# noce2/FluidFramework

Measured on AMD Instinct MI355X. Metric: sequenced merge-tree ops applied/sec (node) at 100k docs; bit-exact text+props, higher is better.
Workload: dtype int32; 1 GPU; c3: 100000 docs/GPU x 10000 sequenced ops, 8 writers, refSeq lag <= 64, insert 0.5 / remove 0.3 / annotate 0.2; docs_total=100000, docs_per_gpu=100000, ops_per_doc=10000, parallelism=doc-shard x1

## Files before the change

### fluidframework_amd/__init__.py

```python
import ctypes

import numpy as np

from . import _native
from .wire import CHECKSUM_DTYPE, OP_DTYPE, Batch, Interner

__all__ = ["MergeTreeBatch", "DeviceBatch", "Batch", "Interner", "DeltaLogOverflow"]


class DeltaLogOverflow(RuntimeError):

    def __init__(self, msg, records):
        super().__init__(msg)
        self.records = records


class PinnedArray:

    def __init__(self, lib, n, dtype):
        dt = np.dtype(dtype)
        nbytes = max(int(n), 1) * dt.itemsize
        self.lib = lib
        self.p = lib.mt_host_alloc(nbytes)
        if not self.p:
# ... 331 lines not shown

    def upload(self, a):
        return DeviceBatch(self, a)

    def generate(self, cfg, doc_base=0, trace=None, ops_per_doc=None, doc_ids=None):
        c = _native.gen_cfg(cfg)
        if ops_per_doc is not None or doc_ids is not None:
            lens = None if ops_per_doc is None else np.ascontiguousarray(ops_per_doc, dtype=np.int32)
            ids = None if doc_ids is None else np.ascontiguousarray(doc_ids, dtype=np.int32)
            for x in (lens, ids):
                if x is not None and x.shape != (self.n_docs,):
                    raise ValueError("ops_per_doc / doc_ids: one per document")
            b = self.lib.mt_generate_docs(self.h, ctypes.byref(c), doc_base, _native.ptr(lens), _native.ptr(ids),
                                          _native.ptr(trace))
        else:
            b = self.lib.mt_generate(self.h, ctypes.byref(c), doc_base, _native.ptr(trace))
        if not b:
            raise RuntimeError(f"mt_generate failed: {self.lib.mt_last_error(self.h).decode()}")
        return DeviceBatch(self, None, handle=b)

    def generated_seeds(self, cfg, doc_base=0, doc_ids=None):
        c = _native.gen_cfg(cfg)
        ids = None if doc_ids is None else np.ascontiguousarray(doc_ids, dtype=np.int32)
        off = np.zeros(self.n_docs + 1, dtype=np.int64)
        self._check(self.lib.mt_generated_seeds_docs(self.h, ctypes.byref(c), doc_base, _native.ptr(ids),
                                                     _native.ptr(off), None), "mt_generated_seeds")
        seed = np.zeros(max(int(off[-1]), 1), dtype=np.uint16)
        self._check(self.lib.mt_generated_seeds_docs(self.h, ctypes.byref(c), doc_base, _native.ptr(ids),
                                                     _native.ptr(off), _native.ptr(seed)), "mt_generated_seeds")
        return off, seed

    def sync(self):
        self._check(self.lib.mt_sync(self.h), "mt_sync")

    def last_hbm_docs(self):
        out = np.zeros(8, dtype=np.uint32)
        self._check(self.lib.mt_last_hbm_docs(self.h, _native.ptr(out)), "mt_last_hbm_docs")
        return dict(total=int(out[0]), spilled=int(out[1]), segments=int(out[2]), blocks=int(out[3]), heap=int(out[4]),
                    text=int(out[5]), props=int(out[6]), at_load=int(out[7]))

    def last_paged_peaks(self):
        out = np.zeros(5, dtype=np.uint32)
        self._check(self.lib.mt_last_paged_peaks(self.h, _native.ptr(out)), "mt_last_paged_peaks")
        return dict(pages=int(out[0]), unsettled=int(out[1]), heap=int(out[2]), segments=int(out[3]),
                    tight_handovers=int(out[4]))

    def last_zamboni(self):
        out = np.zeros(2, dtype=np.uint32)
        self._check(self.lib.mt_last_zamboni(self.h, _native.ptr(out)), "mt_last_zamboni")
        packs = np.zeros(1, dtype=np.uint32)
        self._check(self.lib.mt_last_zamboni_packs(self.h, _native.ptr(packs)), "mt_last_zamboni_packs")
        return {"in_place": int(out[0]), "fallback": int(out[1]), "in_place_packs": int(packs[0])}

    def last_grown(self):
        out = np.zeros(6, dtype=np.uint32)
        self._check(self.lib.mt_last_grown(self.h, _native.ptr(out)), "mt_last_grown")
        return dict(zip(["grown", "rounds", "in_big_region", "pages", "unsettled", "heap"], (int(x) for x in out)))

    def last_kernel_ms(self):
        return float(self.lib.mt_last_kernel_ms(self.h))

    def set_stream_priority(self, priority):
        self._check(self.lib.mt_set_stream_priority(self.h, int(priority)), "mt_set_stream_priority")

    def last_load_ms(self):
        return float(self.lib.mt_last_load_ms(self.h))

    def status(self):
        out = np.zeros(self.n_docs, dtype=np.int32)
        self._check(self.lib.mt_get_status(self.h, _native.ptr(out)), "mt_get_status")
        return out

    def get_length(self, doc):
        out = ctypes.c_uint32()
        self._check(self.lib.mt_get_length(self.h, doc, ctypes.byref(out)), "mt_get_length")
        return out.value

    def get_text(self, doc):
        n = ctypes.c_uint32()
        self._check(self.lib.mt_get_text(self.h, doc, None, 0, ctypes.byref(n)), "mt_get_text")
        buf = np.zeros(max(n.value, 1), dtype=np.uint16)
        self._check(self.lib.mt_get_text(self.h, doc, _native.ptr(buf), n.value, ctypes.byref(n)),
                    "mt_get_text")
        return buf[: n.value].tobytes().decode("utf-16-le", errors="surrogatepass")

    def _text_queries(self, docs, start, end, placeholder):
        if isinstance(placeholder, str):
            units = np.frombuffer(placeholder.encode("utf-16-le", errors="surrogatepass"), dtype=np.uint16)
            if len(units) > 1:
                raise ValueError("get_texts: the placeholder is empty or one UTF-16 unit")
            placeholder = int(units[0]) if len(units) else 0
        if docs is not None:
            docs = np.ascontiguousarray(docs, dtype=np.uint32).reshape(-1)
        n = len(docs) if docs is not None else self.n_docs
        if start is not None:
            start = np.ascontiguousarray(np.broadcast_to(np.asarray(start, dtype=np.int32), (n,)))
        if end is not None:
            end = np.asarray([-1 if e is None else e for e in end] if isinstance(end, (list, tuple)) else end)
            end = np.ascontiguousarray(np.broadcast_to(end.astype(np.int32), (n,)))
        return n, docs, start, end, int(placeholder)

    def get_texts_raw(self, docs=None, start=None, end=None, placeholder=""):
        n, docs, start, end, mu = self._text_queries(docs, start, end, placeholder)
        off = np.zeros(n + 1, dtype=np.int64)
        args = (self.h, n, _native.ptr(docs), _native.ptr(start), _native.ptr(end), mu, _native.ptr(off))
        self._check(self.lib.mt_get_texts(*args, None, 0), "mt_get_texts")
# ... 390 lines not shown
```

### fluidframework_amd/_native.py

```python
import ctypes
import os

import numpy as np

from .wire import CHECKSUM_DTYPE, OP_DTYPE

HERE = os.path.dirname(os.path.abspath(__file__))
MT_E_INVALID, MT_E_HIP, MT_E_NOMEM, MT_E_NODEVICE, MT_E_OVERFLOW, MT_E_STALE_VIEW = -1, -2, -3, -4, -5, -6
LIB_PATH = os.environ.get("MT_LIB_PATH") or os.path.join(HERE, "libmtreplay.so")


class MtOptions(ctypes.Structure):
    _fields_ = [("device", ctypes.c_int32), ("seg_capacity", ctypes.c_int32),
                ("block_capacity", ctypes.c_int32), ("heap_capacity", ctypes.c_int32),
                ("text_capacity", ctypes.c_int32), ("props_capacity", ctypes.c_int32),
                ("delta_log_capacity", ctypes.c_int32), ("lds_seg_capacity", ctypes.c_int32),
                ("page_capacity", ctypes.c_int32), ("page_heap_capacity", ctypes.c_int32),
                ("unsettled_capacity", ctypes.c_int32), ("uid_capacity", ctypes.c_int32),
                ("lds_page_capacity", ctypes.c_int32), ("lds_unsettled_capacity", ctypes.c_int32),
                ("lds_page_heap_capacity", ctypes.c_int32), ("lds_narrow_overlap", ctypes.c_int32),
                ("delta_log_mode", ctypes.c_int32), ("live_client", ctypes.c_int32),
                ("live_group_capacity", ctypes.c_int32), ("paged_slices", ctypes.c_int32),
                ("segment_ordinals", ctypes.c_int32), ("overlap_arena_capacity", ctypes.c_int32)]

# ... 7 lines not shown


REGEN_DTYPE = np.dtype([("kind", "<i4"), ("pos1", "<i4"), ("pos2", "<i4"), ("local_seq", "<i4"),
                        ("text_off", "<u4"), ("text_len", "<u4"), ("props_off", "<u4"), ("flags", "<u4")])


SEG_HIT_DTYPE = np.dtype([("row", "<i4"), ("uid", "<u4"), ("position", "<i4"), ("offset", "<i4"),
                          ("local_position", "<i4"), ("length", "<i4"), ("seq", "<i4"), ("client", "<i4"),
                          ("removed_seq", "<i4"), ("removed_client", "<i4"), ("marker_ref_type", "<i4"),
                          ("flags", "<u4")])
MT_HIT_HOST = 1


class MtGenCfg(ctypes.Structure):
    _fields_ = [("seed", ctypes.c_uint32), ("ops", ctypes.c_int32), ("writers", ctypes.c_int32),
                ("lag", ctypes.c_int32), ("seed_len", ctypes.c_int32), ("text_max", ctypes.c_int32),
                ("n_keys", ctypes.c_int32), ("n_values", ctypes.c_int32),
                ("max_keys_per_op", ctypes.c_int32), ("_pad", ctypes.c_int32),
                ("p_insert", ctypes.c_uint64), ("p_insert_remove", ctypes.c_uint64),
                ("p_newline", ctypes.c_uint64), ("p_len_continue", ctypes.c_uint64),
                ("p_insert_props", ctypes.c_uint64), ("p_null", ctypes.c_uint64)]


_P, _I, _U32, _U64 = ctypes.c_void_p, ctypes.c_int, ctypes.c_uint32, ctypes.c_uint64
SIGNATURES = [
    ("mt_create", _P, [_U32, _P]),
    ("mt_destroy", None, [_P]),
    ("mt_last_error", ctypes.c_char_p, [_P]),
    ("mt_num_docs", _U32, [_P]),
    ("mt_load_initial_text", _I, [_P, _P, _P]),
    ("mt_start_collaboration", _I, [_P, _P, _P]),
    ("mt_reset", _I, [_P]),
    ("mt_apply_ops", _I, [_P, _P, _P, _U64, _P, _U64, _P, _U64]),
    ("mt_load_snapshots", _I, [_P, _P, _P, _P, _U64, _P, _U64, _P, _U64, _P, _P]),
    ("mt_extract_snapshots", _I, [_P, _P, _P, _P, _P, _P, _P]),
    ("mt_snapshots_upload", _P, [_P, _P, _P, _P, _U64, _P, _U64, _P, _U64, _P, _P]),
    ("mt_snapshots_upload_range", _P, [_P, _U32, _U32, _P, _P, _P, _U64, _P, _U64, _P, _U64, _P, _P]),
    ("mt_snapshots_load_async", _I, [_P, _P]),
    ("mt_snapshots_free", None, [_P]),
    ("mt_batch_upload", _P, [_P, _P, _P, _U64, _P, _U64, _P, _U64]),
    ("mt_batch_apply_async", _I, [_P, _P]),
    ("mt_batch_num_ops", _U64, [_P]),
    ("mt_batch_free", None, [_P]),
    ("mt_host_alloc", ctypes.c_void_p, [ctypes.c_uint64]),
    ("mt_host_free", None, [ctypes.c_void_p]),
    ("mt_sync", _I, [_P]),
    ("mt_last_kernel_ms", ctypes.c_float, [_P]),
    ("mt_set_stream_priority", ctypes.c_int, [_P, ctypes.c_int]),
    ("mt_last_load_ms", ctypes.c_float, [_P]),
    ("mt_last_hbm_docs", _I, [_P, _P]),
    ("mt_last_paged_peaks", _I, [_P, _P]),
    ("mt_last_zamboni", _I, [_P, _P]),
    ("mt_last_zamboni_packs", _I, [_P, _P]),
    ("mt_last_grown", _I, [_P, _P]),
    ("mt_generate", _P, [_P, _P, _U32, _P]),
    ("mt_generate_docs", _P, [_P, _P, _U32, _P, _P, _P]),
    ("mt_generated_seeds_docs", _I, [_P, _P, _U32, _P, _P, _P]),
    ("mt_generated_seeds", _I, [_P, _P, _U32, _P, _P]),
    ("mt_batch_sizes", _I, [_P, _P, _P, _P]),
    ("mt_batch_download", _I, [_P, _P, _P, _P, _P]),
    ("mt_get_status", _I, [_P, _P]),
    ("mt_get_length", _I, [_P, _U32, _P]),
    ("mt_get_text", _I, [_P, _U32, _P, _U32, _P]),
    ("mt_get_texts", _I, [_P, _U32, _P, _P, _P, ctypes.c_uint16, _P, _P, _U64]),
    ("mt_get_texts_device", _I, [_P, _U32, _P, _P, _P, ctypes.c_uint16, _P, _P, _U64]),
    ("mt_last_text_ms", _I, [_P, _P]),
    ("mt_get_prop_runs", _I, [_P, _U32, _P, _U32, _P, _P, _U32, _P]),
    ("mt_get_prop_runs_bulk", _I, [_P, _U32, _P, _P, _P, _P, _P, _P, _U64, _P, _U64]),
    ("mt_get_prop_runs_bulk_device", _I, [_P, _U32, _P, _P, _P, _P, _P, _P, _U64, _P, _U64]),
    ("mt_last_props_ms", _I, [_P, _P]),
    ("mt_get_segments", _I, [_P, _U32, _P, _U32, _P, _P, _U32, _P]),
    ("mt_get_segment_props", _I, [_P, _U32, _U32, _P, _U32, _P]),
    ("mt_get_all_segment_props", _I, [_P, _U32, _P, ctypes.c_uint64, _P]),
    ("mt_get_overlap_arena", _I, [_P, _U32, _P]),
    ("mt_get_delta_log", _I, [_P, _U32, _P, _U32, _P]),
    ("mt_delta_log_reset", _I, [_P]),
    ("mt_debug_raw", _I, [_P, _U32, _P, _U32, _P, _P]),
    ("mt_debug_prof", _I, [_P, _P, _I]),
    ("mt_maintenance_counts", _I, [_P, _P]),
    ("mt_checksums", _I, [_P, _P]),
    ("mt_checksums_device", _I, [_P, _P]),
    ("mt_regenerate_pending", _I, [_P, _U32, _P, _U32, _P, _P, _U32, _P, _U32]),
    ("mt_pending_counts", _I, [_P, _P]),
    ("mt_debug_heap", _I, [_P, _U32, _P, _U32, _P, _P, _U32, _P]),
    ("mt_get_containing_segment", _I, [_P, _U32, ctypes.c_int32, ctypes.c_int32, ctypes.c_int32, _P, _P, _U32]),
    ("mt_get_segment_by_uid", _I, [_P, _U32, _U32, ctypes.c_int32, ctypes.c_int32, _P, _P, _U32]),
    ("mt_get_view_lengths", _I, [_P, _U32, _P, _P, _P, _P]),
    ("mt_locate_segments", _I, [_P, _U32, _P, _P, _P, _P, _P]),
    ("mt_locate_uids", _I, [_P, _U32, _P, _P, _P, _P, _P]),
    ("mt_locate_segments_device", _I, [_P, _U32, _P, _P, _P, _P, _P]),
    ("mt_locate_uids_device", _I, [_P, _U32, _P, _P, _P, _P, _P]),
    ("mt_get_view_lengths_bulk", _I, [_P, _U32, _P, _P, _P, _P]),
    ("mt_resolve_remote_positions", _I, [_P, _U32, _P, _P, _P, _P, _P]),
    ("mt_last_locate", _I, [_P, _P, _P]),
]

_lib = None


def load():
    global _lib
    if _lib is not None:
        return _lib
    if not os.path.exists(LIB_PATH):
        raise RuntimeError(f"HIP replay library missing: {LIB_PATH} (run __graft_entry__.build())")
    lib = ctypes.CDLL(LIB_PATH)
# ... 21 lines not shown
```

### fluidframework_amd/csrc/mt_device.h

```cpp
#pragma once
#include <hip/hip_runtime.h>
#include <stdint.h>

#include "../../include/mt_types.h"

#define MT_WAVE 64
#define MT_LV 8
#define MT_MAXN 8
#define MT_HALF 4
#define MT_GRAN 256
#define MT_STATS_WORDS 20
#define MT_ZAMBONI 2
#define MT_KMAX 8
#define MT_PREC (1 + 2 * MT_KMAX)
#define MT_RSEQ_NONE ((int32_t)0x80000000)
#define MT_MARKER_BIT 0x80000000u
#define MT_SCOUR_UNDEF ((int8_t)-1)
#define MT_DOC_RETRY 100

typedef unsigned long long u64;
typedef int v4i __attribute__((ext_vector_type(4)));
typedef unsigned v4u __attribute__((ext_vector_type(4)));
typedef int v2i __attribute__((ext_vector_type(2)));

struct DocHdr {
    int32_t n_seg, depth, heap_n, cur_seq;
    int32_t min_seq, text_top, text_half, props_top;
    int32_t props_half, next_uid, status, dlog_n;
    int32_t n_blk[MT_LV];
    u64 delta_hash;
    int32_t n_ops, pad0;
    int32_t pad[8];
};
static_assert(sizeof(DocHdr) == 128, "DocHdr size");

struct PageMeta {
    uint8_t nseg, nblk;
    uint16_t flg2;
    uint32_t bc;
    int32_t obs;
};
static_assert(sizeof(PageMeta) == 12, "PageMeta size");
static __host__ __device__ inline int pm_bcnt(const PageMeta &m, int q) { return (int)((m.bc >> (4 * q)) & 15u); }
static __host__ __device__ inline int8_t pm_flg(const PageMeta &m, int q) { return (int8_t)((int)((m.flg2 >> (2 * q)) & 3u) - 1); }
#define MT_OSLOTS 64
#define MT_OSLOT_USE 63
#define MT_OVF_BIT (1ull << 63)
#define MT_OVF_HDR 12
static __host__ __device__ inline int mt_ovf_mid(int OA) { return MT_OVF_HDR + (((OA - MT_OVF_HDR) / 2) & ~7); }
#define MT_OVF_ARENA 8192
#define MT_OSLOT_FREE 0x7FFFFFFF
#define MT_PG_SLOTS 64
#define MT_PG_OLB 32
#define HDR_PAGED 0
#define HDR_NPAGES 1
#define HDR_UTN 2
#define HDR_DIAG 3
#define HDR_MSPLIT 4
#define HDR_MAPPEND 5
#define HDR_MUNLINK 6
#define HDR_DLOG_OVF 7

struct PagedRegion {
    v4i *A;
// ... 243 lines not shown
```

### fluidframework_amd/csrc/mt_kernels.h

```cpp
#pragma once
#include "../../include/mt_replay.h"
#include "mt_paged.h"

__device__ static void init_doc_hdr(const DevState &st, int doc, int len) {
    DocHdr h;
    memset(&h, 0, sizeof(h));
    h.depth = 1;
    h.n_blk[0] = 1;
    h.text_top = len;
    h.props_top = 1;
    h.next_uid = 2;
    h.delta_hash = MT_FNV_OFF;
    h.status = len > st.T ? MT_DOC_CAPACITY : 0;
    const size_t S = st.S;
    if (len > 0) {
        h.n_seg = 1;
        st.segA[doc * S] = v4i{len, 0, MT_RSEQ_NONE, pack_cli(-1, 0)};
        st.segO[doc * S] = 0ull;
        st.segB[doc * S] = v4u{0u, 0u, 1u, 0u};
        if (st.segP) {
            u64 *w = (u64 *)(st.segP + doc * S);
            w[0] = w[1] = w[2] = w[3] = 0ull;
        }
    }
// ... 363 lines not shown
    for (int t = 1; t <= g.n && d.status == 0; t++) {
        int r, c, msn;
        gen_pick(g, cfg, t, r, c, msn);
        d.ocs = oslot_of(d, c);
        int vsum = 0;
        for (int base = 0; base < d.n; base += MT_WAVE) {
            const int i = base + lane();
            v4i a;
            u64 o;
            load_ao(d, i, i < d.n, a, o);
            vsum += i < d.n ? view_len(a, o, r, c, d.ocs) : 0;
        }
        const int len = wave_sum(vsum);
        if (dbg_len && lane() == 0) {
            int32_t *q = dbg_len + (g.ob + (t - 1)) * 4;
            q[0] = len;
            q[1] = d.n;
            q[2] = r;
            q[3] = c;
        }
        OpIn in;
        gen_op(g, cfg, t, r, c, msn, len, in, ops_out, text_out, props_out, doc);
        apply_op(d, in, gt, gp);
    }
    gen_end(g, used_out, doc);
    if (T::kLds && d.status == MT_DOC_RETRY) {
        if (lane() == 0) st.retry[doc] = 1;
        return;
    }
    if (lane() == 0) {
        if (d.status) fail_out[doc] = d.status;
        if (!T::kLds) st.retry[doc] = 0;
    }
    store_doc(d, st, doc);
}

template <class T>
__device__ __forceinline__ void pg_peaks(const DevState &st, PagedDoc<T> &pd, int pk_ut, int pk_heap) {
    const int np = nbr(pd.up, 1);
    int ns = 0;
    for (int q = lane(); q < np; q += MT_WAVE) ns += pm_nseg(pd, pd.up.dir[q]);
    ns = wave_sum(ns);
    if (lane() == 0) {
        atomicMax(st.stats + 8, (uint32_t)np);
        atomicMax(st.stats + 9, (uint32_t)pk_ut);
        atomicMax(st.stats + 10, (uint32_t)pk_heap);
        atomicMax(st.stats + 11, (uint32_t)ns);
        if constexpr (pg_zinplace<T>()) {
            const uint32_t zi = pg_zcount(pd)[0], zf = pg_zcount(pd)[1], zp = pg_zcount(pd)[2];
            if (zi) atomicAdd(st.stats + 16, zi);
            if (zf) atomicAdd(st.stats + 17, zf);
            if (zp) atomicAdd(st.stats + 18, zp);
        }
    }
}
#ifndef MT_PAGED_WAVES
#define MT_PAGED_WAVES 3
#endif
#ifndef MT_HM_WAVES
#define MT_HM_WAVES 2
#endif
#ifndef MT_FULL_WAVES
#define MT_FULL_WAVES 2
#endif
#ifndef MT_PACKED_WAVES
#define MT_PACKED_WAVES 2
#endif
template <class T> constexpr int paged_waves() {
    return T::kHM ? MT_HM_WAVES
                  : (T::kMayGrow ? MT_FULL_WAVES : (T::kPacked ? MT_PACKED_WAVES : MT_PAGED_WAVES));
}
#if MT_PAGED_WAVES > 0
#define MT_PAGED_WPE __attribute__((amdgpu_waves_per_eu(paged_waves<T>())))
#else
#define MT_PAGED_WPE
#endif
template <class T>
__device__ __forceinline__ void pg_handover(const DevState &st, int doc, int64_t k, const PagedCaps &pc) {
    if (lane() == 0) {
        st.retry[doc] = pc.tight ? 2 : 3;
        st.resume[doc] = k;
        atomicAdd(st.stats + (pc.tight ? 12 : 13), 1u);
    }
}
struct PagedSlice {
    int64_t ops;
    int skip_lo, skip_hi, cnt_lo, cnt_hi;
};

template <class T>
__global__ void __launch_bounds__(MT_WAVE) MT_PAGED_WPE k_replay_paged(DevState st, const mt_op_rec *ops,
                                                          const int64_t *off, const uint16_t *tin,
                                                          const uint32_t *pin, int use_resume, PagedCaps pc_arg,
                                                          PagedSlice sl) {
    extern __shared__ __attribute__((aligned(16))) uint8_t smem_raw[];
    LDS_AS uint8_t *smem = (LDS_AS uint8_t *)smem_raw;
    const PagedCaps pc = eff_caps<T>(pc_arg);
    const int di = blockIdx.x;
    if (di >= st.n_docs) return;
    if (di >= sl.skip_lo && di < sl.skip_hi) return;
    const int doc = doc_at(st, di);
    if (st.retry[doc] != pc.stage) return;
    if (lane() == 0 && di >= sl.cnt_lo && di < sl.cnt_hi) atomicAdd(st.stats, 1u);
    const PagedLayout L = paged_layout(pc.PP, pc.PH, pc.UT, 0, (int)sizeof(typename T::O_v), T::kPacked, T::kHM);
    const int64_t k0 = use_resume ? st.resume[doc] : off[doc];
    const int64_t kend = off[doc + 1];
// ... 220 lines not shown
```

### fluidframework_amd/csrc/mt_paged.h

```cpp
#pragma once
#include "mt_engine.h"

#ifdef MT_PROF
#define PG_T0(k) const unsigned long long _pt##k = __builtin_amdgcn_s_memtime();
#define PG_T1(k)                                                         \
    if (lane() == 0) {                                                   \
        pd.w.prof[k] += __builtin_amdgcn_s_memtime() - _pt##k;           \
        pd.w.prof[64 + k] += 1ull;                                       \
    }
#define PG_CNT(k)                                                        \
    if (lane() == 0) pd.w.prof[64 + k] += 1ull;
#else
#define PG_T0(k)
#define PG_T1(k)
#define PG_CNT(k)
#endif

template <class T> struct PagedDoc {
    DocT<T> w;
    DocT<T> up;
    LDS_AS PageMeta *meta;
    GLB_AS PageMeta *gmeta;
    LDS_AS int *pvl;
    LDS_AS int *cob;
// ... 13 lines not shown
    GLB_AS uint16_t *goS;
    GLB_AS uint16_t *goL;
    int doc;
    int PP, PH, UT, UM;
    int PPh;
    int ut_n;
    int cur;
    int cur_pos;
    int dirty;
    int tdirty;
    int uid_lo;
    int vvalid, vr, vc;
    int zuid, zpv;
    GLB_AS uint16_t *govf;
    int ovf_top, ovf_last, OA;
    int ovf_maxn, ovf_half;
    uint32_t ovf_made;
    int ovf_peak;
    int press;
    int wgrow, opbound;
    LDS_AS int *sob;
    int sob_ch;
    int wnb, wobs;
};

struct PagedCaps {
    int PP, PH, UT;
    int tight;
    int stage;
    int narrow;
    int grow;
    int packed;
};

#define PW_B 16
#define MT_PK_MASKS 256

struct PagedLayout {
    uint32_t offWA, offWB, offWO, offWcnt, offWflg, offWends, offWscr, offWnb;
    uint32_t offUcnt, offUnb, offDir, offMeta, offCob, offHeap, offUpage, offUA, offUO, offGen, offProf,
        total;
};
static __host__ __device__ inline PagedLayout paged_layout(int PP, int PH, int UT, int gen_words, int ob,
                                                           bool packed = false, bool hm = false) {
    PagedLayout L;
    uint32_t o = 0;
    L.offWA = o; o += 16u * MT_PG_SLOTS;
    L.offWB = o; o += 16u * MT_PG_SLOTS;
    L.offWO = o; o += (uint32_t)ob * MT_PG_SLOTS;
    L.offUA = o; o += (packed ? 12u : 16u) * UT;
    o = (o + 7u) & ~7u;
    L.offUO = o; o += packed ? 8u * MT_PK_MASKS + MT_PK_MASKS / 8 : ((((uint32_t)ob * UT) + 7u) & ~7u);
    L.offHeap = o; o += 8u * (PH + 1);
    L.offMeta = o; o += hm ? 0u : (uint32_t)sizeof(PageMeta) * PP + 12u;
    L.offUpage = o; o += packed ? 0u : (2u * UT + 3u) & ~3u;
    L.offCob = o; o += hm ? 8u * (uint32_t)((PP + 63) / 64) + 4u * 64 : 4u * PP;
    L.offWscr = o; o += 64u * 4;
    L.offWnb = o; o += MT_LV * 4;
    L.offUnb = o; o += MT_LV * 4;
    L.offGen = o; o += 4u * gen_words;
    L.offDir = o; o += 2u * PP;
    L.offWends = o; o += 2u * PW_B;
    L.offWcnt = o; o += (uint32_t)MT_LV * PW_B;
    L.offWflg = o; o += PW_B;
    L.offUcnt = o; o += (uint32_t)(pcnt_bytes(PP) - PP);
#ifdef MT_PROF
    o = (o + 7u) & ~7u;
    L.offProf = o; o += 128u * 8;
#else
    L.offProf = 0;
#endif
    L.total = (o + 15u) & ~15u;
    return L;
}

TD PagedDoc<T> &pdoc(DocT<T> &w) { return *reinterpret_cast<PagedDoc<T> *>(&w); }
template <class T> __device__ __forceinline__ PagedCaps eff_caps(PagedCaps pc) {
    if constexpr (T::kPP > 0) pc.PP = T::kPP;
    if constexpr (T::kPH > 0) pc.PH = T::kPH;
    if constexpr (T::kUT > 0) pc.UT = T::kUT;
    return pc;
}
TD void pg_fail_cap(DocT<T> &w, int cause) {
    if (w.status == 0) w.cap_cause = cause;
    fail(w, MT_DOC_CAPACITY);
}
__device__ __forceinline__ PageMeta pm_load(const LDS_AS PageMeta *m) {
    PageMeta r;
    r.nseg = m->nseg;
    r.nblk = m->nblk;
    r.flg2 = m->flg2;
    r.bc = m->bc;
    r.obs = m->obs;
    return r;
}
__device__ __forceinline__ int pm_bcnt_l(const LDS_AS PageMeta *m, int q) { return (int)((m->bc >> (4 * q)) & 15u); }
__device__ __forceinline__ int8_t pm_flg_l(const LDS_AS PageMeta *m, int q) {
    return (int8_t)((int)((m->flg2 >> (2 * q)) & 3u) - 1);
}
TD int pm_nseg(const PagedDoc<T> &pd, int pg) {
    if constexpr (T::kHM) {
        gsync_rd();
        return pd.gmeta[pg].nseg;
    } else {
        return pd.meta[pg].nseg;
    }
}
TD int pm_nblk(const PagedDoc<T> &pd, int pg) {
    if constexpr (T::kHM) {
// ... 1177 lines not shown
            pd.gO[(size_t)npg * MT_PG_SLOTS + t] = o;
            pd.gB[(size_t)npg * MT_PG_SLOTS + t] = b;
            const uint32_t uid = b.z & ~MT_MARKER_BIT;
            if (uid < (uint32_t)pd.UM) pd.gumap[uid] = (uint16_t)npg;
            ol = obs_len(a);
            add = unsettled<T>(a, w.min_seq);
        }
        const u64 am = ballot(add);
        if (pd.ut_n + __popcll(am) > pd.UT) {
            pg_fail_cap(w, 8);
            return;
        }
        const int mi = tab_midx(pd, add && o != 0);
        if (mi < 0) {
            pg_fail_cap(w, 8);
            return;
        }
        if (add) tab_put(pd, pd.ut_n + __popcll(am & ((1ull << lane()) - 1ull)), c0 + m, a, o, mi);
        pd.ut_n += __popcll(am);
        const int obs = wave_sum(ol);
        const bool vb = lane() >= blo && lane() < bhi;
        pm_set_blocks(pd, npg, lane() - blo, vb, bcnt, bflg);
        if (lane() == 0) {
            pm_set_ns(pd, npg, s_hi - s_lo, bhi - blo);
            pm_set_obs(pd, npg, obs);
        }
        wsync<T>();
    }
    for (int j = 0; j < nch; j++) {
        const int pg = uni(up.dir[c0 + j]);
        if (lane() == 0) pm_set_ns(pd, pg, 0, 0);
        wsync<T>();
    }
    blk_replace(up, 1, c0, nch, k, base, extra);
    if (up.status) {
        pg_fail_cap(w, 7);
        return;
    }
    for (int m = 0; m < k; m++)
        if (lane() == 0) up.dir[c0 + m] = (uint16_t)newp[m];
    if (lane() == 0) lvl(up, 2)[P] = (uint8_t)k;
    wsync<T>();
    pg_cob_rebuild(pd);
    int top_l = 2, top_b = P;
    if (k < MT_HALF && 3 < up.depth) pack_counts(up, 2, P, top_l, top_b);
    if (up.status) {
        if (w.status == 0) w.cap_cause = up.cap_cause;
        fail(w, MT_DOC_INTERNAL);
        return;
    }
    if (ordon(w)) ord_canon(up, top_l, top_b);
}

TD LDS_AS uint32_t *pg_zcount(PagedDoc<T> &pd) { return (LDS_AS uint32_t *)(pd.meta + pd.PP); }
template <class T> constexpr bool pg_zinplace() {
#ifdef MT_NO_ZINPLACE
    return false;
#else
    return !T::kLog && !T::kHM && !T::kLive;
#endif
}
template <class T> constexpr bool pg_zpack() {
#ifdef MT_NO_ZPACK
    return false;
#else
    return pg_zinplace<T>();
#endif
}
__device__ __forceinline__ int lane_push(int v, int dst) { return __builtin_amdgcn_ds_permute(dst << 2, v); }
TD bool pg_pack_inplace(PagedDoc<T> &pd, int pg, v4i a, v4u b, const ScourPlan &pl, uint32_t bc, int q, int bstart) {
    DocT<T> &w = pd.w;
    const int k = lane();
    const int n = uni(pm_nseg(pd, pg)), nb = uni(pm_nblk(pd, pg));
    const int cnt = pm_bc_of(bc, q);
    const int keep = __popcll(pl.m_surv);
    const int n1 = n - (cnt - keep);
    if (nb > 8) return true;
    const bool in = k >= bstart && k < bstart + cnt;
    const u64 below = (1ull << k) - 1ull;
    const ScourGroups g1 = scour_groups(a, in, pl.m_join, pl.m_surv);
    v4i a1 = a;
    v4u b1 = b;
    if (g1.m_grp) {
        const uint32_t lastw = (uint32_t)__shfl((int)b.w, g1.gend & (MT_WAVE - 1), MT_WAVE);
        if ((g1.m_grp >> k) & 1ull) {
            a1.x = g1.glen;
            b1.w = lastw & (SEGF_NL_KNOWN | SEGF_NL);
        }
    }
    const int d1 = k < bstart ? k
                   : !in      ? k - (cnt - keep)
                   : ((pl.m_surv >> k) & 1ull) ? bstart + __popcll(pl.m_surv & below) : MT_WAVE - 1;
    a1 = v4i{lane_push(a1.x, d1), lane_push(a1.y, d1), lane_push(a1.z, d1), lane_push(a1.w, d1)};
    b1 = v4u{(uint32_t)lane_push((int)b1.x, d1), (uint32_t)lane_push((int)b1.y, d1),
             (uint32_t)lane_push((int)b1.z, d1), (uint32_t)lane_push((int)b1.w, d1)};
    const int src1 = lane_push(k, d1);
    const bool in2 = k < n1;
    int start2 = 0;
    {
        int st = 0;
        for (int j = 0; j < nb; j++) {
            if (k >= st) start2 = st;
            st += j == q ? keep : pm_bc_of(bc, j);
        }
    }
    bool nl2;
    const ScourPlan p2 = scour_plan(w, a1, b1, in2, false, start2, nl2);
// ... 272 lines not shown
    int start;
    int ostart;
    int pos = pg_find(pd, op.pos1, false, start, ostart);
    if constexpr (T::kLog) {
        const int np = nbr(pd.up, 1);
        if (pos < 0 && slen == 0 && np > 0 && !(op.flags & MT_F_LOAD)) {
            pos = np - 1;
            const int lp = uni((int)pd.up.dir[pos]);
            start -= pg_page_view(pd, pos);
            ostart -= uni(pm_obs(pd, lp));
        }
    }
    if (pos < 0) {
        if (slen == 0) {
            if (op.flags & MT_F_LOAD) return;
            Cb cb = cb_begin(w, op.seq, MT_OP_INSERT);
            cb.n = 1;
            cb_log(w, -1);
            cb_log(w, 0);
            cb.h = fnv_u64(cb.h, fnv_u32(fnv_u32(MT_FNV_OFF, (uint32_t)-1), 0u));
            cb_end(w, cb);
            return;
        }
        fail(w, MT_DOC_INSERT_FAILED);
        return;
    }
    pg_load_pos(pd, pos, ostart);
    if (w.status) return;
    OpIn rel = in;
    rel.op.pos1 = op.pos1 - start;
    pd.vvalid = 0;
    pd.tdirty = 1;
    op_insert(w, rel, tin, pin);
    if (w.status) return;
    pg_win_sync(pd);
    if (T::kLog && w.dfr_rec >= 0) pg_log_deferred(pd);
}

TD void pg_boundary(PagedDoc<T> &pd, int p, int r, int c) {
    pg_views_cached(pd, r, c);
    if (pd.w.status) return;
    int start;
    int ostart;
    const int pos = pg_find(pd, p, true, start, ostart);
    if (pos < 0 || start >= p) return;
    pg_load_pos(pd, pos, ostart);
    if (pd.w.status) return;
    pd.tdirty = 1;
    boundary(pd.w, p - start, r, c);
    if (pd.w.status) return;
    pg_win_sync(pd);
}

TD void pg_op_range(PagedDoc<T> &pd, const mt_op_rec &op, const GLB_AS uint32_t *pin) {
    DocT<T> &w = pd.w;
    const int r = op.ref_seq, c = op_cli(op), p1 = op.pos1, p2 = op.pos2;
    const bool rem = op.kind == MT_OP_REMOVE;
    const GLB_AS uint32_t *rec = (!rem && op.props != MT_NO_PROPS) ? pin + op.props : nullptr;
    if (rec && (rec[0] >> 16) == MT_COMBINE_OTHER) {
        fail(w, MT_DOC_UNSUPPORTED);
        return;
    }
    if (!rec) rec = (const GLB_AS uint32_t *)&kEmptyPropsRec;
    pg_boundary(pd, p1, r, c);
    if (w.status) return;
    pg_boundary(pd, p2, r, c);
    if (w.status) return;
    Cb cb = cb_begin(w, op.seq, op.kind);
    pg_views_cached(pd, r, c);
    if (w.status) return;
    pd.vvalid = 0;
    int start;
    int ostart;
    int pos = pg_find(pd, p1, true, start, ostart);
    if (pos >= 0) {
        int carry = start, ocarry = ostart;
        const int np = nbr(pd.up, 1);
        while (pos < np && carry < p2) {
            pg_load_pos(pd, pos, ocarry);
            if (w.status) return;
            pd.tdirty = 1;
            PG_T0(45)
            const bool done = range_mark(w, op, rec, carry, ocarry, cb);
            PG_T1(45)
            if (w.status) return;
            pg_win_sync(pd);
            if (w.status) return;
            if (done) break;
            pos = pg_cur_pos(pd) + 1;
        }
    }
    cb_end(w, cb);
}

TD void pg_renumber(PagedDoc<T> &pd, bool soft = false) {
    DocT<T> &w = pd.w;
    pg_win_flush(pd);
    if (w.status) return;
    pd.cur = -1;
    pd.cur_pos = -1;
    pd.vvalid = 0;
    gsync();
    const int np = nbr(pd.up, 1);
    if (2 * pd.PP > w.T_cap) {
        pg_fail_cap(w, 4);
        return;
    }
    GLB_AS int32_t *first = (GLB_AS int32_t *)text_base(w, 1 - w.text_half);
    int carry = 1;
    for (int base = 0; base < np; base += MT_WAVE) {
        const int q = base + lane();
        const int pg = q < np ? (int)pd.up.dir[q] : 0;
        const int ns = q < np ? pm_nseg(pd, pg) : 0;
        const int inc = wave_scan_incl(ns);
        if (q < np) first[pg] = carry + inc - ns;
        carry += bcast(inc, MT_WAVE - 1);
    }
    gsync();
    gsync_rd();
    const int i = lane();
// ... 605 lines not shown
    w.paged = 1;
    w.obs_base = 0;
    w.pend_split = 0;
    w.pend_second = -1;
    w.dir = nullptr;
    up = w;
    up.paged = 0;
    up.cnt = smem + L.offUcnt - pc.PP;
    up.nb = (LDS_AS int32_t *)(smem + L.offUnb);
    up.dir = (LDS_AS uint16_t *)(smem + L.offDir);
    up.B_cap = pc.PP;
    up.status = 0;
    if (ordon(w)) {
        up.ob = (GLB_AS uint16_t *)tier_paged<T::kBig>(st, doc).oU;
        up.obst = pd.PPh;
    }
    pd.pvl = (LDS_AS int *)(smem + L.offCob);
    pd.cob = pd.pvl;
    pd.cdl = pd.cob + (pc.PP + 63) / 64;
    if constexpr (T::kHM) {
        pd.meta = nullptr;
        pd.gmeta = (GLB_AS PageMeta *)tier_paged<T::kBig>(st, doc).meta;
        pd.sob = pd.cdl + (pc.PP + 63) / 64;
        pd.sob_ch = -1;
        pd.wnb = pd.wobs = 0;
    } else {
        pd.meta = (LDS_AS PageMeta *)(smem + L.offMeta);
    }
    pd.vgen = 0;
    pd.scr_ch = -1;
    pd.upage = (LDS_AS uint16_t *)(smem + L.offUpage);
    pd.uA = (LDS_AS v4i *)(smem + L.offUA);
    pd.uO = (LDS_AS typename T::O_v *)(smem + L.offUO);
    if constexpr (T::kPacked) {
        pd.uL = (LDS_AS uint32_t *)(smem + L.offUA);
        pd.uS = pd.uL + pc.UT;
        pd.uP = pd.uS + pc.UT;
        pd.sbase = h.cur_seq - 32000;
        pd.uM = (LDS_AS u64 *)(smem + L.offUO);
        pd.mbm = (LDS_AS uint32_t *)(smem + L.offUO + 8u * MT_PK_MASKS);
        if (lane() < MT_PK_MASKS / 32) pd.mbm[lane()] = lane() == 0 ? 1u : 0u;
        if (lane() == 0) pd.uM[0] = 0;
    }
    pd.cur = -1;
    pd.cur_pos = -1;
    pd.dirty = 0;
    pd.tdirty = 0;
    pd.vvalid = 0;
    pd.wgrow = 0;
    pd.opbound = 0;
    pd.zuid = 0;
    pd.zpv = 0;
    pd.press = 0;
    if constexpr (!T::kHM) {
        if (lane() == 0) pg_zcount(pd)[0] = pg_zcount(pd)[1] = pg_zcount(pd)[2] = 0;
    }
    pd.ovf_top = MT_OVF_HDR;
    pd.ovf_last = 0;
    pd.ovf_maxn = 0;
    pd.ovf_half = 0;
    pd.ovf_made = 0;
    pd.ovf_peak = 0;
    if constexpr (T::kOvf) {
        if (pd.govf) {
            const GLB_AS uint32_t *hw = (const GLB_AS uint32_t *)pd.govf;
            pd.ovf_top = max((int)hw[0], MT_OVF_HDR);
            pd.ovf_last = (int)hw[1];
            pd.ovf_maxn = (int)hw[2];
            pd.ovf_made = hw[4];
            pd.ovf_peak = (int)hw[5];
            pd.ovf_half = ((int)hw[3] & 1) && pd.ovf_top > mt_ovf_mid(pd.OA) ? 1 : 0;
        }
    }
}

TD void pg_mark_free(PagedDoc<T> &pd) {
    const int np = nbr(pd.up, 1);
    pd.vvalid = 0;
    for (int base = 0; base < pd.PP; base += MT_WAVE)
        if (base + lane() < pd.PP) pm_set_nblk(pd, base + lane(), pm_nblk(pd, base + lane()) | 0x80);
    wsync<T>();
    for (int base = 0; base < np; base += MT_WAVE)
        if (base + lane() < np) {
            const int pg = pd.up.dir[base + lane()];
            pm_set_nblk(pd, pg, pm_nblk(pd, pg) & 0x7F);
        }
    wsync<T>();
    for (int base = 0; base < pd.PP; base += MT_WAVE) {
        const int pg = base + lane();
        if (pg < pd.PP && (pm_nblk(pd, pg) & 0x80)) pm_set_ns(pd, pg, 0, 0);
    }
    wsync<T>();
}

TD bool pg_load(PagedDoc<T> &pd, const DevState &st) {
    const PgCold g = pg_cold<T>(st, pd.doc);
    DocT<T> &w = pd.w;
    DocT<T> &up = pd.up;
    const DocHdr h = *w.hp;
    const int np = h.n_blk[1];
    if (np > pd.PP || h.pad[HDR_UTN] > pd.UT || h.heap_n > pd.PH) return false;
    for (int l = 2; l < h.depth; l++)
        if (h.n_blk[l] + 4 > pcnt_cap(pd.PP, l)) return false;
    if (T::kOvlBits < 64 && w.wide) return false;
    if constexpr (!T::kOvf) {
        if (pd.govf) {
            const GLB_AS uint32_t *hw = (const GLB_AS uint32_t *)pd.govf;
            if ((int)hw[0] > MT_OVF_HDR && (int)hw[1] > w.min_seq) return false;
        }
// ... 270 lines not shown
```

### fluidframework_amd/csrc/mt_replay.hip

```cpp
#include <hip/hip_runtime.h>

#include <algorithm>
#include <cstdlib>
#include <cstdio>
#include <cstring>
#include <string>
#include <vector>

#include "../../include/mt_replay.h"
#include "mt_kernels.h"
#include "mt_variants.h"
#ifdef MT_SINGLE_TU
#define MT_VARIANT_DEF(n, k) const void *mtk_##n() { return (const void *)k; }
MT_VARIANTS(MT_VARIANT_DEF)
#endif

__global__ void __launch_bounds__(MT_WAVE) k_init(DevState st, const int64_t *seed_off,
                                                  const uint16_t *seed) {
    const int doc = blockIdx.x;
    if (doc >= st.n_docs) return;
    oslot_reset(st, doc);
    if (st.bslot && lane() == 0) st.bslot[doc] = -1;
    const int64_t s0 = seed_off ? seed_off[doc] : 0, s1 = seed_off ? seed_off[doc + 1] : 0;
    const int len = (int)(s1 - s0);
// ... 2131 lines not shown
    HIPCHK(h, hipStreamCreateWithPriority(&s, hipStreamNonBlocking,
                                          priority > 0 ? greatest : (priority < 0 ? least : 0)));
    hipStreamDestroy(h->stream);
    h->stream = s;
    return 0;
}

int mt_last_hbm_docs(mt_handle *h, uint32_t *out) {
    if (!h || !out) return MT_E_INVALID;
    HIPCHK(h, hipSetDevice(h->device));
    SETTLE(h);
    HIPCHK(h, hipMemcpy(out, h->st.stats, 8 * sizeof(uint32_t), hipMemcpyDeviceToHost));
    return 0;
}

int mt_last_grown(mt_handle *h, uint32_t *out) {
    if (!h || !out) return MT_E_INVALID;
    SETTLE(h);
    uint32_t in_big = 0;
    for (int32_t x : h->bslot_h) in_big += x >= 0;
    out[0] = h->grown_last;
    out[1] = h->grow_rounds_last;
    out[2] = in_big;
    out[3] = (uint32_t)h->big_caps.PP;
    out[4] = (uint32_t)h->big_caps.UT;
    out[5] = (uint32_t)h->big_caps.PH;
    return 0;
}

int mt_last_paged_peaks(mt_handle *h, uint32_t *out) {
    if (!h || !out) return MT_E_INVALID;
    HIPCHK(h, hipSetDevice(h->device));
    SETTLE(h);
    HIPCHK(h, hipMemcpy(out, h->st.stats + 8, 5 * sizeof(uint32_t), hipMemcpyDeviceToHost));
    return 0;
}

int mt_last_zamboni(mt_handle *h, uint32_t *out) {
    if (!h || !out) return MT_E_INVALID;
    HIPCHK(h, hipSetDevice(h->device));
    SETTLE(h);
    HIPCHK(h, hipMemcpy(out, h->st.stats + 16, 2 * sizeof(uint32_t), hipMemcpyDeviceToHost));
    return 0;
}

int mt_last_zamboni_packs(mt_handle *h, uint32_t *out) {
    if (!h || !out) return MT_E_INVALID;
    HIPCHK(h, hipSetDevice(h->device));
    SETTLE(h);
    HIPCHK(h, hipMemcpy(out, h->st.stats + 18, sizeof(uint32_t), hipMemcpyDeviceToHost));
    return 0;
}

int mt_apply_ops(mt_handle *h, const int64_t *doc_op_off, const mt_op_rec *ops, uint64_t n_ops,
                 const uint16_t *text, uint64_t text_len, const uint32_t *props,
                 uint64_t props_len) {
    if (!h) return MT_E_INVALID;
    h->err.clear();
    mt_batch *b = mt_batch_upload(h, doc_op_off, ops, n_ops, text, text_len, props, props_len);
    if (!b) return h->err.rfind("mt_batch_upload: device", 0) == 0 ? MT_E_NOMEM : MT_E_INVALID;
    int rc = mt_batch_apply_async(h, b);
    if (rc == 0) rc = mt_sync(h);
    mt_batch_free(b);
    return rc;
}

struct mt_snapshots {
    int device = 0;
    uint32_t doc_lo = 0, n_docs = 0;
    int64_t *off = nullptr;
    int32_t *nh = nullptr, *min_seq = nullptr, *cur_seq = nullptr;
    mt_seg_rec *segs = nullptr;
    uint16_t *text = nullptr;
    uint32_t *props = nullptr;
    mt_batch *body = nullptr;
    LoadScratch sc = {nullptr, nullptr, nullptr, nullptr, nullptr, nullptr};
    int64_t *sc_off = nullptr;
    bool any_big = false;
};

void mt_snapshots_free(mt_snapshots *s) {
    if (!s) return;
    hipSetDevice(s->device);
    void *ps[] = {s->off, s->nh, s->min_seq, s->cur_seq, s->segs, s->text, s->props, s->sc.A, s->sc.O, s->sc.B,
                  s->sc.cnt, s->sc.flg, s->sc_off};
    for (void *p : ps)
        if (p) hipFree(p);
    mt_batch_free(s->body);
    delete s;
}

mt_snapshots *mt_snapshots_upload_range(mt_handle *h, uint32_t doc_lo, uint32_t n_docs, const int64_t *doc_seg_off,
                                        const int32_t *n_header, const mt_seg_rec *segs, uint64_t n_segs,
                                        const uint16_t *text, uint64_t text_len, const uint32_t *props,
                                        uint64_t props_len, const int32_t *min_seq, const int32_t *cur_seq) {
    if (!h || !doc_seg_off || !n_header || !min_seq || !cur_seq || (n_segs && !segs)) return nullptr;
    if (n_docs == 0 || doc_lo > h->n_docs || n_docs > h->n_docs - doc_lo) {
        h->err = "mt_snapshots_upload_range: documents [doc_lo, doc_lo + n_docs) outside the handle (or empty)";
        return nullptr;
    }
    const uint32_t N = n_docs;
    for (uint32_t d = 0; d < N; d++)
        if (n_header[d] < 0 || doc_seg_off[d] + n_header[d] > doc_seg_off[d + 1] ||
            doc_seg_off[d + 1] > (int64_t)n_segs) {
            h->err = "mt_snapshots_upload: bad document segment ranges";
            return nullptr;
// ... 1644 lines not shown
```

### include/mt_replay.h

```cpp
#ifndef MT_REPLAY_H
#define MT_REPLAY_H
#include <stddef.h>
#include <stdint.h>

#include "mt_types.h"

#ifdef __cplusplus
extern "C" {
#endif

#define MT_E_INVALID (-1)
#define MT_E_HIP (-2)
#define MT_E_NOMEM (-3)
#define MT_E_NODEVICE (-4)
#define MT_E_OVERFLOW (-5)
#define MT_E_STALE_VIEW (-6)

typedef struct mt_handle mt_handle;
typedef struct mt_batch mt_batch;

typedef struct mt_options {
    int32_t device;
    int32_t seg_capacity;
    int32_t block_capacity;
// ... 22 lines not shown
    uint32_t seed;
    int32_t ops, writers, lag, seed_len, text_max, n_keys, n_values, max_keys_per_op;
    int32_t _pad;
    uint64_t p_insert, p_insert_remove, p_newline, p_len_continue, p_insert_props, p_null;
} mt_gen_cfg;

mt_handle *mt_create(uint32_t n_docs, const mt_options *opt);
void mt_destroy(mt_handle *h);
const char *mt_last_error(const mt_handle *h);
uint32_t mt_num_docs(const mt_handle *h);

int mt_load_initial_text(mt_handle *h, const int64_t *seed_off, const uint16_t *seed_text);
int mt_reset(mt_handle *h);
int mt_start_collaboration(mt_handle *h, const int32_t *min_seq, const int32_t *cur_seq);

int mt_apply_ops(mt_handle *h, const int64_t *doc_op_off, const mt_op_rec *ops, uint64_t n_ops,
                 const uint16_t *text, uint64_t text_len, const uint32_t *props,
                 uint64_t props_len);

int mt_load_snapshots(mt_handle *h, const int64_t *doc_seg_off, const int32_t *n_header, const mt_seg_rec *segs,
                      uint64_t n_segs, const uint16_t *text, uint64_t text_len, const uint32_t *props,
                      uint64_t props_len, const int32_t *min_seq, const int32_t *cur_seq);
typedef struct mt_snapshots mt_snapshots;
mt_snapshots *mt_snapshots_upload(mt_handle *h, const int64_t *doc_seg_off, const int32_t *n_header,
                                  const mt_seg_rec *segs, uint64_t n_segs, const uint16_t *text, uint64_t text_len,
                                  const uint32_t *props, uint64_t props_len, const int32_t *min_seq,
                                  const int32_t *cur_seq);
mt_snapshots *mt_snapshots_upload_range(mt_handle *h, uint32_t doc_lo, uint32_t n_docs, const int64_t *doc_seg_off,
                                        const int32_t *n_header, const mt_seg_rec *segs, uint64_t n_segs,
                                        const uint16_t *text, uint64_t text_len, const uint32_t *props,
                                        uint64_t props_len, const int32_t *min_seq, const int32_t *cur_seq);
int mt_snapshots_load_async(mt_handle *h, const mt_snapshots *s);
void mt_snapshots_free(mt_snapshots *s);
float mt_last_load_ms(mt_handle *h);

int mt_extract_snapshots(mt_handle *h, int64_t *io, mt_seg_rec *recs, uint16_t *text, uint32_t *props,
                         int32_t *min_seq, int32_t *cur_seq);

mt_batch *mt_batch_upload(mt_handle *h, const int64_t *doc_op_off, const mt_op_rec *ops,
                          uint64_t n_ops, const uint16_t *text, uint64_t text_len,
                          const uint32_t *props, uint64_t props_len);
int mt_batch_apply_async(mt_handle *h, const mt_batch *b);
uint64_t mt_batch_num_ops(const mt_batch *b);
void mt_batch_free(mt_batch *b);
void *mt_host_alloc(uint64_t bytes);
void mt_host_free(void *p);
int mt_sync(mt_handle *h);
float mt_last_kernel_ms(const mt_handle *h);
int mt_set_stream_priority(mt_handle *h, int priority);
int mt_last_hbm_docs(mt_handle *h, uint32_t *out);
int mt_last_paged_peaks(mt_handle *h, uint32_t *out);
int mt_last_zamboni(mt_handle *h, uint32_t *out);
int mt_last_zamboni_packs(mt_handle *h, uint32_t *out);

int mt_last_grown(mt_handle *h, uint32_t *out);

mt_batch *mt_generate(mt_handle *h, const mt_gen_cfg *cfg, uint32_t doc_index_base,
                      int32_t *view_len_trace );
mt_batch *mt_generate_docs(mt_handle *h, const mt_gen_cfg *cfg, uint32_t doc_index_base,
                           const int32_t *ops_per_doc, const int32_t *doc_ids, int32_t *view_len_trace);
int mt_generated_seeds_docs(mt_handle *h, const mt_gen_cfg *cfg, uint32_t doc_index_base, const int32_t *doc_ids,
                            int64_t *seed_off, uint16_t *seed_text);
int mt_generated_seeds(mt_handle *h, const mt_gen_cfg *cfg, uint32_t doc_index_base,
                       int64_t *seed_off, uint16_t *seed_text);
int mt_batch_sizes(const mt_batch *b, uint64_t *n_ops, uint64_t *text_len, uint64_t *props_len);
int mt_batch_download(const mt_batch *b, int64_t *doc_op_off, mt_op_rec *ops, uint16_t *text,
                      uint32_t *props);

int mt_get_status(mt_handle *h, int32_t *out_status);
int mt_get_length(mt_handle *h, uint32_t doc, uint32_t *out);
int mt_get_text(mt_handle *h, uint32_t doc, uint16_t *out, uint32_t cap, uint32_t *out_len);
int mt_get_texts(mt_handle *h, uint32_t n, const uint32_t *docs, const int32_t *start,
                 const int32_t *end, uint16_t marker_unit, int64_t *off, uint16_t *out, uint64_t cap);
int mt_get_texts_device(mt_handle *h, uint32_t n, const uint32_t *docs, const int32_t *start,
                        const int32_t *end, uint16_t marker_unit, void *off_dev, void *out_dev, uint64_t cap);
int mt_last_text_ms(mt_handle *h, float *out );
int mt_get_prop_runs(mt_handle *h, uint32_t doc, uint32_t *runs, uint32_t cap_runs,
                     uint32_t *n_runs, uint32_t *records, uint32_t cap_words,
                     uint32_t *n_words);
int mt_get_prop_runs_bulk(mt_handle *h, uint32_t n, const uint32_t *docs, const int32_t *start,
                          const int32_t *end, int64_t *run_off , int64_t *word_off ,
                          uint32_t *runs, uint64_t cap_runs, uint32_t *records, uint64_t cap_words);
int mt_get_prop_runs_bulk_device(mt_handle *h, uint32_t n, const uint32_t *docs, const int32_t *start,
                                 const int32_t *end, void *run_off_dev, void *word_off_dev,
                                 void *runs_dev, uint64_t cap_runs, void *records_dev, uint64_t cap_words);
int mt_last_props_ms(mt_handle *h, float *out );
int mt_get_segments(mt_handle *h, uint32_t doc, int32_t *rows, uint32_t cap_rows,
                    uint32_t *n_rows, int32_t *leaves, uint32_t cap_leaves, uint32_t *n_leaves);
int mt_get_overlap_arena(mt_handle *h, uint32_t doc, int32_t *out );
int mt_get_all_segment_props(mt_handle *h, uint32_t doc, int32_t *out, uint64_t cap_words, uint64_t *n_words);
int mt_get_segment_props(mt_handle *h, uint32_t doc, uint32_t seg_index, uint32_t *pairs,
                         uint32_t cap_pairs, int32_t *n_pairs);
typedef struct mt_seg_info {
    int32_t row;
    uint32_t uid;
    int32_t position;
    int32_t offset;
    int32_t length;
    int32_t seq, client;
    int32_t removed_seq;
    int32_t removed_client;
    int32_t marker_ref_type;
    int32_t text_len;
    int32_t ordinal_len;
    uint16_t ordinal[16];
} mt_seg_info;
// ... 61 lines not shown
```

Measured before the change: 167.4 million ops/s.

## Add single-page fast path for range ops in paged replay

For remove/annotate range ops whose whole span falls within one page, the code loads that page once, splits at both ends locally and marks the range, instead of running two independent page boundary lookups followed by a general range walk. It falls back to the general path when a split is pending or the range spans pages. It also adds counters to LDS stats and a host query for path counts, which costs extra atomics and a few LDS words per doc.

After: 171.2 million ops/s, median of 6. 1.02x the previous value.

```diff
diff --git a/fluidframework_amd/__init__.py b/fluidframework_amd/__init__.py
--- a/fluidframework_amd/__init__.py
+++ b/fluidframework_amd/__init__.py
@@ -407,6 +407,11 @@
         self._check(self.lib.mt_last_zamboni_packs(self.h, _native.ptr(packs)), "mt_last_zamboni_packs")
         return {"in_place": int(out[0]), "fallback": int(out[1]), "in_place_packs": int(packs[0])}
 
+    def last_range_paths(self):
+        out = np.zeros(3, dtype=np.uint32)
+        self._check(self.lib.mt_last_range_paths(self.h, _native.ptr(out)), "mt_last_range_paths")
+        return {"one_page": int(out[0]), "split_fallback": int(out[1]), "general": int(out[2])}
+
     def last_grown(self):
         out = np.zeros(6, dtype=np.uint32)
         self._check(self.lib.mt_last_grown(self.h, _native.ptr(out)), "mt_last_grown")
diff --git a/fluidframework_amd/_native.py b/fluidframework_amd/_native.py
--- a/fluidframework_amd/_native.py
+++ b/fluidframework_amd/_native.py
@@ -83,6 +83,7 @@
     ("mt_last_paged_peaks", _I, [_P, _P]),
     ("mt_last_zamboni", _I, [_P, _P]),
     ("mt_last_zamboni_packs", _I, [_P, _P]),
+    ("mt_last_range_paths", _I, [_P, _P]),
     ("mt_last_grown", _I, [_P, _P]),
     ("mt_generate", _P, [_P, _P, _U32, _P]),
     ("mt_generate_docs", _P, [_P, _P, _U32, _P, _P, _P]),
diff --git a/fluidframework_amd/csrc/mt_device.h b/fluidframework_amd/csrc/mt_device.h
--- a/fluidframework_amd/csrc/mt_device.h
+++ b/fluidframework_amd/csrc/mt_device.h
@@ -9,7 +9,7 @@
 #define MT_MAXN 8
 #define MT_HALF 4
 #define MT_GRAN 256
-#define MT_STATS_WORDS 20
+#define MT_STATS_WORDS 24
 #define MT_ZAMBONI 2
 #define MT_KMAX 8
 #define MT_PREC (1 + 2 * MT_KMAX)
diff --git a/fluidframework_amd/csrc/mt_kernels.h b/fluidframework_amd/csrc/mt_kernels.h
--- a/fluidframework_amd/csrc/mt_kernels.h
+++ b/fluidframework_amd/csrc/mt_kernels.h
@@ -439,6 +439,10 @@
             if (zf) atomicAdd(st.stats + 17, zf);
             if (zp) atomicAdd(st.stats + 18, zp);
         }
+        const uint32_t r1 = pg_zcount(pd)[3], rs = pg_zcount(pd)[4], rg = pg_zcount(pd)[5];
+        if (r1) atomicAdd(st.stats + 20, r1);
+        if (rs) atomicAdd(st.stats + 21, rs);
+        if (rg) atomicAdd(st.stats + 22, rg);
     }
 }
 #ifndef MT_PAGED_WAVES
diff --git a/fluidframework_amd/csrc/mt_paged.h b/fluidframework_amd/csrc/mt_paged.h
--- a/fluidframework_amd/csrc/mt_paged.h
+++ b/fluidframework_amd/csrc/mt_paged.h
@@ -89,9 +89,9 @@
     o = (o + 7u) & ~7u;
     L.offUO = o; o += packed ? 8u * MT_PK_MASKS + MT_PK_MASKS / 8 : ((((uint32_t)ob * UT) + 7u) & ~7u);
     L.offHeap = o; o += 8u * (PH + 1);
-    L.offMeta = o; o += hm ? 0u : (uint32_t)sizeof(PageMeta) * PP + 12u;
+    L.offMeta = o; o += hm ? 0u : (uint32_t)sizeof(PageMeta) * PP + 24u;
     L.offUpage = o; o += packed ? 0u : (2u * UT + 3u) & ~3u;
-    L.offCob = o; o += hm ? 8u * (uint32_t)((PP + 63) / 64) + 4u * 64 : 4u * PP;
+    L.offCob = o; o += hm ? 8u * (uint32_t)((PP + 63) / 64) + 4u * 64 + 24u : 4u * PP;
     L.offWscr = o; o += 64u * 4;
     L.offWnb = o; o += MT_LV * 4;
     L.offUnb = o; o += MT_LV * 4;
@@ -1375,7 +1375,10 @@
     if (ordon(w)) ord_canon(up, top_l, top_b);
 }
 
-TD LDS_AS uint32_t *pg_zcount(PagedDoc<T> &pd) { return (LDS_AS uint32_t *)(pd.meta + pd.PP); }
+TD LDS_AS uint32_t *pg_zcount(PagedDoc<T> &pd) {
+    if constexpr (T::kHM) return (LDS_AS uint32_t *)(pd.sob + 64);
+    return (LDS_AS uint32_t *)(pd.meta + pd.PP);
+}
 template <class T> constexpr bool pg_zinplace() {
 #ifdef MT_NO_ZINPLACE
     return false;
@@ -1754,6 +1757,13 @@
     pg_win_sync(pd);
 }
 
+template <class T> constexpr bool pg_range1() {
+#ifdef MT_NO_RANGE1
+    return false;
+#else
+    return !T::kLog && !T::kHM && !T::kLive;
+#endif
+}
 TD void pg_op_range(PagedDoc<T> &pd, const mt_op_rec &op, const GLB_AS uint32_t *pin) {
     DocT<T> &w = pd.w;
     const int r = op.ref_seq, c = op_cli(op), p1 = op.pos1, p2 = op.pos2;
@@ -1764,10 +1774,63 @@
         return;
     }
     if (!rec) rec = (const GLB_AS uint32_t *)&kEmptyPropsRec;
-    pg_boundary(pd, p1, r, c);
-    if (w.status) return;
-    pg_boundary(pd, p2, r, c);
-    if (w.status) return;
+    int step = 0;
+    if constexpr (pg_range1<T>()) {
+        pg_views_cached(pd, r, c);
+        if (w.status) return;
+        int start;
+        int ostart;
+        const int pos = pg_find(pd, p1, true, start, ostart);
+        if (pos >= 0 && p1 < p2 && p2 < start + uni(pd.pvl[pos])) {
+            if (lane() == 0) pg_zcount(pd)[3]++;
+            pg_load_pos(pd, pos, ostart);
+            if (w.status) return;
+            pd.tdirty = 1;
+            const int n0 = w.n;
+            if (start < p1) {
+                boundary(w, p1 - start, r, c);
+                if (w.status) return;
+                if (w.pend_split) step = 1;
+            }
+            if (step == 0) {
+                boundary(w, p2 - start, r, c);
+                if (w.status) return;
+                if (w.pend_split) step = 2;
+            }
+            if (step == 0) {
+                if (w.n != n0 && !rem && w.props_top + MT_WAVE > w.P_cap) {
+                    pg_win_sync(pd);
+                    if (w.status) return;
+                }
+                Cb cb = cb_begin(w, op.seq, op.kind);
+                pd.vvalid = 0;
+                int carry = start, ocarry = ostart;
+                PG_T0(45)
+                range_mark(w, op, rec, carry, ocarry, cb);
+                PG_T1(45)
+                if (w.status) return;
+                pg_win_sync(pd);
+                if (w.status) return;
+                cb_end(w, cb);
+                return;
+            }
+            if (lane() == 0) pg_zcount(pd)[4]++;
+            pg_win_sync(pd);
+            if (w.status) return;
+        } else {
+            if (lane() == 0) pg_zcount(pd)[5]++;
+        }
+    } else {
+        if (lane() == 0) pg_zcount(pd)[5]++;
+    }
+    if (step < 1) {
+        pg_boundary(pd, p1, r, c);
+        if (w.status) return;
+    }
+    if (step < 2) {
+        pg_boundary(pd, p2, r, c);
+        if (w.status) return;
+    }
     Cb cb = cb_begin(w, op.seq, op.kind);
     pg_views_cached(pd, r, c);
     if (w.status) return;
@@ -2479,9 +2542,7 @@
     pd.zuid = 0;
     pd.zpv = 0;
     pd.press = 0;
-    if constexpr (!T::kHM) {
-        if (lane() == 0) pg_zcount(pd)[0] = pg_zcount(pd)[1] = pg_zcount(pd)[2] = 0;
-    }
+    if (lane() < 6) pg_zcount(pd)[lane()] = 0;
     pd.ovf_top = MT_OVF_HDR;
     pd.ovf_last = 0;
     pd.ovf_maxn = 0;
diff --git a/fluidframework_amd/csrc/mt_replay.hip b/fluidframework_amd/csrc/mt_replay.hip
--- a/fluidframework_amd/csrc/mt_replay.hip
+++ b/fluidframework_amd/csrc/mt_replay.hip
@@ -2207,6 +2207,15 @@
     return 0;
 }
 
+int mt_last_range_paths(mt_handle *h, uint32_t *out) {
+    if (!h || !out) return MT_E_INVALID;
+    HIPCHK(h, hipSetDevice(h->device));
+    SETTLE(h);
+    HIPCHK(h, hipMemcpy(out, h->st.stats + 20, 3 * sizeof(uint32_t), hipMemcpyDeviceToHost));
+    out[0] -= out[1];
+    return 0;
+}
+
 int mt_apply_ops(mt_handle *h, const int64_t *doc_op_off, const mt_op_rec *ops, uint64_t n_ops,
                  const uint16_t *text, uint64_t text_len, const uint32_t *props,
                  uint64_t props_len) {
diff --git a/include/mt_replay.h b/include/mt_replay.h
--- a/include/mt_replay.h
+++ b/include/mt_replay.h
@@ -98,6 +98,7 @@
 int mt_last_paged_peaks(mt_handle *h, uint32_t *out);
 int mt_last_zamboni(mt_handle *h, uint32_t *out);
 int mt_last_zamboni_packs(mt_handle *h, uint32_t *out);
+int mt_last_range_paths(mt_handle *h, uint32_t out[3]);
 
 int mt_last_grown(mt_handle *h, uint32_t *out);
 
```
